# brantburnett/Snappier

Measured on AMD Instinct MI355X. Metric: uncompressed GB/s block compress+decompress, 64 KiB blocks, higher is better.
Workload: dtype u8

## Files before the change

include/snappier_hip.h:

```cpp
#ifndef SNAPPIER_HIP_H
#define SNAPPIER_HIP_H

#include <stddef.h>
#include <stdint.h>

#ifdef __cplusplus
extern "C" {
#endif

typedef enum snp_status {
    SNP_OK = 0,
    SNP_ERR_OUTPUT_TOO_SMALL = 1,
    SNP_ERR_BAD_OFFSET = 2,
    SNP_ERR_TOO_LONG = 3,
    SNP_ERR_INCOMPLETE = 4,
    SNP_ERR_BAD_LENGTH = 5,
    SNP_ERR_CRC_MISMATCH = 6,
    SNP_ERR_CHUNK_TYPE = 7,
    SNP_ERR_OVERLAP = 8,
    SNP_ERR_BAD_ARG = 9,
    SNP_ERR_DEVICE = 10,
    SNP_ERR_TRUNCATED_STREAM = 11
} snp_status;

// ... 31 lines not shown
    SNP_OPT_PARALLEL_DECODE_MIN = 8,
    SNP_OPT_FENCED = 9,
    SNP_OPT_DECODE_LEFTOVERS = 10,
    SNP_OPT_CRC_KERNEL = 11,
    SNP_OPT_COMPRESS_WINDOW_POSITIONS = 12,
    SNP_OPT_COMPRESS_WINDOW_GLOBAL_MIN_BATCH = 13,
    SNP_OPT_COMPRESS_LANE_STORES = 14,
    SNP_OPT_COMPRESS_LANE_PROBES = 15,
    SNP_OPT_COMPRESS_LANES_PER_WAVEFRONT = 16,
    SNP_OPT_COMPRESS_SLICE = 17,
    SNP_OPT_COMPRESS_SMALL_INPUT_LDS = 18,
    SNP_OPT_COMPRESS_SMALL_INPUT_LANES = 19,
    SNP_OPT_FRAME_SCAN = 20,
    SNP_OPT_DECODE_LDS_THROTTLE = 21,
    SNP_OPT_COMPRESS_WINDOW_GLOBAL_SLOTS = 22,
    SNP_OPT_COMPRESS_WINDOW_DUAL_MIN_BATCH = 23
} snp_option;
#define SNP_OPT_CRC_TABLE_FREE SNP_OPT_CRC_KERNEL
snp_status snp_ctx_set_option(snp_ctx* ctx, int option, int64_t value);
snp_status snp_ctx_get_option(const snp_ctx* ctx, int option, int64_t* out_value);
snp_status snp_ctx_reserve_compress(snp_ctx* ctx, uint32_t nfragments);
const char* snp_status_string(int status);
const char* snp_version(void);


int64_t snp_max_compressed_length(int64_t n);
int64_t snp_max_fragment_compressed_length(int64_t n);
snp_status snp_get_uncompressed_length(const uint8_t* in, size_t n, uint32_t* out_len, uint32_t* out_header_bytes);


snp_status snp_try_compress(snp_ctx* ctx, const uint8_t* in, size_t n, uint8_t* out, size_t cap, size_t* written);
// ... 50 lines not shown
```

snappier_amd/_native.py:

```python
from __future__ import annotations

import ctypes as C
import os
import re

import torch

HERE = os.path.dirname(os.path.abspath(__file__))
LIB_PATH = os.environ.get("SNAPPIER_HIP_LIB") or os.path.join(HERE, "libsnappier_hip.so")
HEADER_PATH = os.path.join(HERE, "..", "include", "snappier_hip.h")

(OK, ERR_OUTPUT_TOO_SMALL, ERR_BAD_OFFSET, ERR_TOO_LONG, ERR_INCOMPLETE, ERR_BAD_LENGTH, ERR_CRC_MISMATCH,
 ERR_CHUNK_TYPE, ERR_OVERLAP, ERR_BAD_ARG, ERR_DEVICE, ERR_TRUNCATED_STREAM) = range(12)
HASH_CRC32C, HASH_MUL = 0, 1
BLOCK_SIZE = 65536
MAX_BLOCK_COMPRESSED = 76491
(OPT_DECODE_LAYOUT, OPT_SMALL_BLOCK_MAX, OPT_SMALL_BLOCK_MIN_BATCH, OPT_COMPRESS_LAYOUT, OPT_COMPRESS_WINDOW_MAX_BATCH,
 OPT_TABLE_PROBE_TRIES, OPT_TABLE_PROBE_MAX_BYTES, OPT_PARALLEL_DECODE_MIN, OPT_FENCED, OPT_DECODE_LEFTOVERS, OPT_CRC_KERNEL,
 OPT_COMPRESS_WINDOW_POSITIONS, OPT_COMPRESS_WINDOW_GLOBAL_MIN_BATCH, OPT_COMPRESS_LANE_STORES, OPT_COMPRESS_LANE_PROBES,
 OPT_COMPRESS_LANES_PER_WAVEFRONT, OPT_COMPRESS_SLICE, OPT_COMPRESS_SMALL_INPUT_LDS, OPT_COMPRESS_SMALL_INPUT_LANES, OPT_FRAME_SCAN,
 OPT_DECODE_LDS_THROTTLE, OPT_COMPRESS_WINDOW_GLOBAL_SLOTS, OPT_COMPRESS_WINDOW_DUAL_MIN_BATCH) = range(1, 24)
OPT_CRC_TABLE_FREE = OPT_CRC_KERNEL
DECODE_AUTO, DECODE_WAVE_ONLY, DECODE_SMALL_LANES, DECODE_SMALL_TEAM4, DECODE_SMALL_TEAM8, DECODE_SMALL_TEAM16, DECODE_SERIAL = range(7)
COMPRESS_AUTO, COMPRESS_LANES, COMPRESS_WINDOW_LDS, COMPRESS_WINDOW_GLOBAL, COMPRESS_WINDOW_DUAL = 0, 2, 3, 4, 5


def declared_symbols(header: str = HEADER_PATH) -> list[str]:
    with open(header) as f:
        text = f.read()
    text = re.sub(r"/\*.*?\*/", "", text, flags=re.S)
    return sorted(set(re.findall(r"\b(snp_[a-z0-9_]+)\s*\(", text)))


_lib = None
_lab = None
LAB_PATH = os.path.join(HERE, "variants", "libsnappier_hip_lab.so")
# ... 198 lines not shown
```

snappier_amd/csrc/capi_batch.hip:

```cpp
#include "capi_internal.h"

#ifndef SNP_W_DUAL_LDS_PER_CU
#define SNP_W_DUAL_LDS_PER_CU 4u
#endif

bool snp_ctx::launch_decompress(const u8* d_in, const u64* in_off, const u32* in_len, u32 nblocks, u8* d_out, const u64* out_off,
                       const u32* out_cap, u32* out_len, i32* status, const u8* chunk_type)
{
    if (small_max && nblocks >= small_min_blocks && decode_layout == 0 && !no_prepass) {
        const u32 sub_cap = nblocks / 64 + 128;
        if (!ensure(redo, (static_cast<size_t>(sub_cap) * 64 + 128) * 4, "hipMalloc(redo list)")) return false;
        u32* const ctl = static_cast<u32*>(redo.p);
        u32* const list = ctl + 128;
        const bool capturing = stream_is_capturing();
        RelaxedCaptureMode relaxed;
        if (capturing) {
        } else if (hint && hint_ev && hint_pending && hipEventQuery(hint_ev) == hipSuccess) {
            hint_pending = false;
            if (hint_from_prepass) {
                u64 left = 0;
                for (int k = 0; k < 64; ++k) left += hint[k];
                hint_mostly_large = left * 2 > hint_blocks;
            } else if (hint[67]) {
                hint_mostly_large = static_cast<u64>(hint[65]) * 2 < hint[67];
// ... 105 lines not shown
    }
    const bool capturing = stream_is_capturing();
    if (capturing) {
    } else if (chint && chint_ev && chint_pending && hipEventQuery(chint_ev) == hipSuccess) {
        chint_pending = false;
        chint_small = chint[0] != 0 && chint[0] <= 512;
        chint_mid = chint[0] != 0 && chint[0] <= 4096;
        chint_tiny = (chint[0] > 80 && chint[0] <= 768) ? static_cast<int>((chint[0] + 15u) >> 4) : 0;
    } else {
        (void)hipGetLastError();
    }
    const u32 kSlice = slice_fragments;
    if (!ensure(small, 256, "hipMalloc(scalars)") || !borrow_tables(nblocks < kSlice ? nblocks : kSlice)) return false;
    snp_lane_tuning tune = lane_tune;
    tune.hint = (chint_small ? 32 : 0) | (chint_mid ? 256 : 0) | (chint_tiny << 9);
    for (u32 first = 0; first < nblocks; first += kSlice) {
        const u32 cnt = nblocks - first < kSlice ? nblocks - first : kSlice;
        if (!check(snp_launch_compress_lanes(d_in, in_off + first, in_len + first, cnt, d_out, out_off + first,
                                             out_len + first, status + first, variant, emit_varint, &tp,
                                             static_cast<u32*>(small.p), stream, &tune),
                   "compress (lanes) launch")) {
            return_tables();
            return false;
        }
    }
    return_tables();
    if (!capturing && chint_ready() && !chint_pending) {
        if (hipMemcpyAsync(chint, small.p, 4, hipMemcpyDeviceToHost, stream) == hipSuccess && hipEventRecord(chint_ev, stream) == hipSuccess)
            chint_pending = true;
        else
            (void)hipGetLastError();
    }
    return true;
}

bool snp_ctx::side_stream_ready()
{
    if (side_state) return side_state > 0;
    side_state = -1;
    RelaxedCaptureMode relaxed;
    if (hipStreamCreateWithFlags(&side_stream, hipStreamNonBlocking) != hipSuccess) { (void)hipGetLastError(); side_stream = nullptr; return false; }
    for (auto& e : side_ev)
        if (hipEventCreateWithFlags(&e, hipEventDisableTiming) != hipSuccess) { (void)hipGetLastError(); return false; }
    side_state = 1;
    return true;
}

bool snp_ctx::chint_ready()
{
    if (!chint && hipHostMalloc(reinterpret_cast<void**>(&chint), 64, hipHostMallocDefault) != hipSuccess) { (void)hipGetLastError(); chint = nullptr; return false; }
    if (!chint_ev && hipEventCreateWithFlags(&chint_ev, hipEventDisableTiming) != hipSuccess) { (void)hipGetLastError(); chint_ev = nullptr; return false; }
    return true;
}

extern "C" {


snp_status snp_compress_batch(snp_ctx* c, const uint8_t* in, const uint64_t* in_off, const uint32_t* in_len,
                              uint32_t nblocks, uint8_t* out, const uint64_t* out_off, uint32_t* out_len,
                              int32_t* status)
{
    if (!c || (nblocks && (!in || !in_off || !in_len || !out || !out_off || !out_len || !status))) return SNP_ERR_BAD_ARG;
// ... 39 lines not shown
```

snappier_amd/csrc/capi_ctx.hip:

```cpp
#include "capi_internal.h"

bool snp_ctx::check(hipError_t e, const char* what)
{
    if (e == hipSuccess) return true;
    err = std::string(what) + ": " + hipGetErrorString(e);
    return false;
}

bool snp_ctx::ensure(DevBuf& b, size_t bytes, const char* what)
{
    if (bytes <= b.cap) return true;
    if (stream_is_capturing()) {
        err = std::string(what) + ": a workspace would have to grow while the stream is being captured -- make the same call once before the capture (or snp_ctx_reserve_compress)";
        return false;
    }
    if (b.p) {
        if (was_captured) kept.push_back(b.p);
        else (void)hipFree(b.p);
    }
    b.p = nullptr;
    b.cap = 0;
    size_t want = bytes + bytes / 4 + 4096;
    if (!check(hipMalloc(&b.p, want), what)) return false;
    b.cap = want;
// ... 103 lines not shown
    }
    c->pool = snp_pool_of(device);
    if (!c->pool) { if (c->own_stream) (void)hipStreamDestroy(c->stream); delete c; return SNP_ERR_DEVICE; }
    {
        std::lock_guard<std::mutex> g(c->pool->mu);
        ++c->pool->users;
    }
    c->fenced = 1 | 8;
#ifdef SNAPPIER_HIP_DEBUG_ENV
    snp_apply_debug_env(c);
#endif
    *out_ctx = c;
    return SNP_OK;
}

uint64_t snp_ctx_counter(const snp_ctx* c, int which) { return (c && which >= 0 && which < 7) ? c->counters[which] : 0; }

snp_status snp_ctx_reserve_compress(snp_ctx* c, uint32_t nfragments)
{
    if (!c) return SNP_ERR_BAD_ARG;
    if (nfragments == 0) return SNP_OK;
    DevGuard dg(c);
    if (!dg.ok) return SNP_ERR_DEVICE;
    if (!c->borrow_tables(nfragments < c->slice_fragments ? nfragments : c->slice_fragments, true)) return SNP_ERR_DEVICE;
    c->return_tables();
    return SNP_OK;
}

snp_status snp_ctx_set_option(snp_ctx* c, int option, int64_t v)
{
    if (!c) return SNP_ERR_BAD_ARG;
// ... 79 lines not shown
        case SNP_OPT_COMPRESS_SMALL_INPUT_LANES:
            if (v != 0 && v != 16 && v != 32 && v != 64) return SNP_ERR_BAD_ARG;
            c->lane_tune.small_lanes = static_cast<int>(v);
            return SNP_OK;
        case SNP_OPT_FRAME_SCAN:
            if (v != 0 && v != 1) return SNP_ERR_BAD_ARG;
            c->frame_scan = static_cast<int>(v);
            return SNP_OK;
        case SNP_OPT_COMPRESS_WINDOW_GLOBAL_SLOTS:
            if (v < 0 || v > 65536) return SNP_ERR_BAD_ARG;
            c->win_gslots = static_cast<u32>(v);
            return SNP_OK;
        case SNP_OPT_COMPRESS_WINDOW_DUAL_MIN_BATCH:
            if (v < 0 || v > 0xffffffffll) return SNP_ERR_BAD_ARG;
            c->win_dual_min = static_cast<u32>(v);
            return SNP_OK;
        case SNP_OPT_DECODE_LDS_THROTTLE:
            if (v < 0 || v > 65536) return SNP_ERR_BAD_ARG;
            c->dec_lds = static_cast<int>(v / 256 * 256);
            return SNP_OK;
        default:
            return SNP_ERR_BAD_ARG;
    }
}

snp_status snp_ctx_get_option(const snp_ctx* c, int option, int64_t* out)
{
    if (!c || !out) return SNP_ERR_BAD_ARG;
    switch (option) {
        case SNP_OPT_DECODE_LAYOUT: *out = (c->fenced & 2) ? 6 : c->no_prepass ? 1 : c->small_lanes ? 2 : c->small_team_log ? c->small_team_log + 1 : 0; return SNP_OK;
// ... 7 lines not shown
        case SNP_OPT_FENCED: *out = c->fenced & 1; return SNP_OK;
        case SNP_OPT_DECODE_LEFTOVERS: *out = c->redo_grid ? 1 : c->redo_list ? 2 : 0; return SNP_OK;
        case SNP_OPT_CRC_KERNEL: *out = c->crc_kernel; return SNP_OK;
        case SNP_OPT_COMPRESS_WINDOW_POSITIONS: *out = c->win_np; return SNP_OK;
        case SNP_OPT_COMPRESS_WINDOW_GLOBAL_MIN_BATCH: *out = c->win_gtab_min; return SNP_OK;
        case SNP_OPT_COMPRESS_LANE_STORES: *out = c->lane_tune.opts; return SNP_OK;
        case SNP_OPT_COMPRESS_LANE_PROBES: *out = c->lane_tune.probes; return SNP_OK;
        case SNP_OPT_COMPRESS_LANES_PER_WAVEFRONT: *out = c->lane_tune.lanes_per_wave; return SNP_OK;
        case SNP_OPT_COMPRESS_SLICE: *out = c->slice_fragments; return SNP_OK;
        case SNP_OPT_COMPRESS_SMALL_INPUT_LDS: *out = c->lane_tune.small_bytes; return SNP_OK;
        case SNP_OPT_COMPRESS_SMALL_INPUT_LANES: *out = c->lane_tune.small_lanes; return SNP_OK;
        case SNP_OPT_FRAME_SCAN: *out = c->frame_scan; return SNP_OK;
        case SNP_OPT_DECODE_LDS_THROTTLE: *out = c->dec_lds; return SNP_OK;
        case SNP_OPT_COMPRESS_WINDOW_GLOBAL_SLOTS: *out = c->win_gslots; return SNP_OK;
        case SNP_OPT_COMPRESS_WINDOW_DUAL_MIN_BATCH: *out = c->win_dual_min; return SNP_OK;
        default: return SNP_ERR_BAD_ARG;
    }
}

void snp_ctx_destroy(snp_ctx* c)
{
    if (!c) return;
    {
        DevGuard dg(c);
        (void)hipStreamSynchronize(c->stream);
        for (DevBuf* b : {&c->in, &c->out, &c->meta, &c->work, &c->fragtab, &c->scan, &c->small, &c->redo, &c->win_tables, &c->own_tables})
            if (b->p) (void)hipFree(b->p);
        for (void* q : c->kept) (void)hipFree(q);
        if (c->pool) {
            std::lock_guard<std::mutex> g(c->pool->mu);
            if (--c->pool->users == 0) c->pool->destroy();
        }
        if (c->order_ev) (void)hipEventDestroy(c->order_ev);
        if (c->hint_ev) (void)hipEventDestroy(c->hint_ev);
        if (c->chint_ev) (void)hipEventDestroy(c->chint_ev);
        if (c->chint) (void)hipHostFree(c->chint);
        if (c->hint) (void)hipHostFree(c->hint);
        if (c->copy_stream) { (void)hipStreamSynchronize(c->copy_stream); (void)hipStreamDestroy(c->copy_stream); }
        if (c->side_stream) { (void)hipStreamSynchronize(c->side_stream); (void)hipStreamDestroy(c->side_stream); }
        for (auto& e : c->side_ev) if (e) (void)hipEventDestroy(e);
        for (auto& e : c->copy_ev) if (e) (void)hipEventDestroy(e);
        if (c->own_stream) (void)hipStreamDestroy(c->stream);
    }
    delete c;
}

snp_status snp_ctx_set_stream(snp_ctx* c, void* stream)
{
    if (!c) return SNP_ERR_BAD_ARG;
    DevGuard dg(c);
    if (!dg.ok) return SNP_ERR_DEVICE;
    hipStream_t next = static_cast<hipStream_t>(stream);
    if (c->own_stream) {
        (void)hipStreamSynchronize(c->stream);
        (void)hipStreamDestroy(c->stream);
// ... 70 lines not shown
```

snappier_amd/csrc/capi_internal.h:

```cpp
#pragma once
#include <hip/hip_runtime.h>

#include <cstdio>
#include <cstring>
#include <new>
#include <algorithm>
#include <cmath>
#include <chrono>
#include <mutex>
#include <string>
#include <utility>
#include <vector>

#include "snp_rules.h"

struct ChunkRows {
    u8* type;
    u64 *body_off, *out_off;
    u32 *body_len, *crc, *out_cap, *out_len, *tag;
    i32* status;
};

extern "C" {
hipError_t snp_launch_decompress(const u8*, const u64*, const u32*, u32, u8*, const u64*, const u32*, u32*, i32*,
                                 const u8*, int, hipStream_t, const u32*);
u32 snp_tag_index_entries(u32, u32);
size_t snp_tag_index_workspace_bytes(u32, u32);
size_t snp_tag_index_fallback_offset(u32, u32);
hipError_t snp_launch_tag_index(const u8*, u32, u32, u32, u64*, u64*, u32*, u64*, u32*, u32*, hipStream_t);
u32 snp_tag_index_chunks_ready(u32, u32, u64);
hipError_t snp_launch_tag_index_begin(u64*, u32, u32, int, hipStream_t);
int snp_tag_index_look_back_only(u32, u32);
hipError_t snp_launch_tag_index_chunks(const u8*, u32, u32, u64*, u32, u32, hipStream_t);
hipError_t snp_launch_tag_index_finish(const u8*, u32, u32, u32, u64*, u64*, u32*, u64*, u32*, u32*, hipStream_t);
hipError_t snp_launch_compress_win(const u8*, const u64*, const u32*, u32, u8*, const u64*, u32*, i32*, int, int, int,
                                   hipStream_t, uint16_t*, u32);
size_t snp_compress_win_table_bytes(u32);
hipError_t snp_launch_compress_win_dual(const u8*, const u64*, const u32*, u32, u8*, const u64*, u32*, i32*, int, int, hipStream_t, hipStream_t,
                                        hipEvent_t, hipEvent_t, uint16_t*, u32, u32, u32*);
hipError_t snp_launch_decompress_small(const u8*, const u64*, const u32*, u32, u8*, const u64*, const u32*, u32*, i32*, const u8*,
                                       u32, hipStream_t, u32*, u32*, u32, u32);
hipError_t snp_launch_sample_caps(const u32*, u32, u32, u32*, hipStream_t);
hipError_t snp_launch_decompress_list(const u8*, const u64*, const u32*, u32, u8*, const u64*, const u32*, u32*, i32*, const u8*, int,
                                      hipStream_t, const u32*, u32*, u32, u32);
hipError_t snp_launch_compress_lanes(const u8*, const u64*, const u32*, u32, u8*, const u64*, u32*, i32*, int, int, const snp_table_pieces*,
                                     u32*, hipStream_t, const snp_lane_tuning*);
size_t snp_compress_lanes_workspace(u32);
hipError_t snp_probe_tables(const snp_table_pieces*, u32, u32, hipStream_t, float*);
hipError_t snp_launch_crc32c(const u8*, const u64*, const u32*, u32, int, u32*, const u32*, i32*, hipStream_t);
hipError_t snp_launch_gather(const u8*, const u64*, const u32*, u8*, const u64*, u32, hipStream_t);
hipError_t snp_launch_frame_chunks(u64, u32, u64, u64*, u32*, u64*, hipStream_t);
hipError_t snp_launch_frame_plan(const u32*, const u32*, u32, u8*, u32*, u64*, u64*, hipStream_t);
hipError_t snp_launch_frame_header_only(u8*, u64*, hipStream_t);
hipError_t snp_launch_frame_scan(const u8*, u64, u64, u32, const ChunkRows&, u64*, hipStream_t);
// ... 58 lines not shown
    int crc_kernel = 0;
    int crc_bits() const { return crc_kernel == 1 ? 2 : crc_kernel == 2 ? 4 : 0; }
    bool no_prepass = false;
    bool small_lanes = false;
    bool redo_grid = false, redo_list = false;
    u32 small_team_log = 0;
    u32 slice_fragments = 262144;
    u32 win_gtab_min = 4096;
    u32 win_gslots = 0;
    u32 win_dual_min = 1536;
    hipStream_t side_stream = nullptr;
    hipEvent_t side_ev[2] = {nullptr, nullptr};
    int side_state = 0;
    bool side_stream_ready();
    u32 win_max = 32768;
    snp_lane_tuning lane_tune{0, -1, 0, -1, 0, 0};
    DevBuf in, out, meta, work, fragtab, scan, small, redo, win_tables;
    int frame_scan = 0;
    uint64_t counters[7] = {0, 0, 0, 0, 0, 0, 0};
    bool table_tries_set = false;
    std::string err;

    bool launch_decompress(const u8* d_in, const u64* in_off, const u32* in_len, u32 nblocks, u8* d_out, const u64* out_off,
                           const u32* out_cap, u32* out_len, i32* status, const u8* chunk_type);
    bool launch_compress(const u8* d_in, const u64* in_off, const u32* in_len, u32 nblocks, u8* d_out, const u64* out_off,
                         u32* out_len, i32* status, int emit_varint);
    bool decode_chunks(const u8* d_in, const ChunkRows& r, u32 n, u8* d_out);
    u32* hint = nullptr;
    hipEvent_t hint_ev = nullptr;
    bool hint_pending = false, hint_mostly_large = false, hint_from_prepass = false, hint_seen = false;
    u32 hint_blocks = 0, hint_mean_cap = 256;
    bool hint_ready();
    u32 n_waves = 0;
    u32 persistent_waves();
// ... 49 lines not shown
```

snappier_amd/csrc/compress_lanes.hip:

```cpp
#include <cstdlib>

#include "snp_device.h"

#ifndef SNP_CL_FLAT
#define SNP_CL_FLAT 1
#endif
#ifndef SNP_CL_SLOTS
#define SNP_CL_SLOTS 1
#endif

namespace {

constexpr u32 kDefaultSlots = SNP_CL_SLOTS;

constexpr u32 crc_step32(u32 x)
{
    for (int k = 0; k < 32; ++k) x = (x >> 1) ^ ((x & 1u) ? 0x82F63B78u : 0u);
    return x;
}

__device__ __forceinline__ u32 check_bits(u32 bytes) { return (bytes * 0x9E3779B1u) & 0xffff0000u; }

__device__ __forceinline__ u32 table_swap(u32* p, u32 v) { return __hip_atomic_exchange(p, v, __ATOMIC_RELAXED, __HIP_MEMORY_SCOPE_AGENT); }

// ... 562 lines not shown

namespace {
__global__ void k_debug_lane_match_length(const u8* buf, u32 n, u32 s1, u32 s2, u32* out)
{
    if (threadIdx.x == 0) *out = lane_find_match_length(buf, s1, s2, n);
}
}
extern "C" int snp_debug_lane_match_length(const u8* d_buf, u32 n, u32 s1, u32 s2, u32* d_out, hipStream_t stream)
{
    hipLaunchKernelGGL(k_debug_lane_match_length, dim3(1), dim3(SNP_WAVE), 0, stream, d_buf, n, s1, s2, d_out);
    return static_cast<int>(hipGetLastError());
}

extern "C" size_t snp_compress_lanes_workspace(u32 nblocks) { return static_cast<size_t>(nblocks) * 16384u * sizeof(u32); }

__global__ __launch_bounds__(256) void k_max_len(const u32* __restrict__ in_len, u32 nblocks, u32* __restrict__ max_len)
{
    u32 m = 0;
    for (u32 i = blockIdx.x * 256 + threadIdx.x; i < nblocks; i += gridDim.x * 256) m = max(m, in_len[i]);
    for (int sh = 32; sh >= 1; sh >>= 1) m = max(m, static_cast<u32>(__shfl_xor(static_cast<int>(m), sh, 64)));
    if ((threadIdx.x & 63u) == 0) atomicMax(max_len, m);
}

extern "C" hipError_t snp_launch_compress_lanes(const u8* in, const u64* in_off, const u32* in_len, u32 nblocks, u8* out,
                                                const u64* out_off, u32* out_len, i32* status, int variant,
                                                int emit_varint, const snp_table_pieces* tables, u32* max_len, hipStream_t stream, const snp_lane_tuning* tune)
{
    if (nblocks == 0) return hipSuccess;
    hipError_t e = snp_zero_words_async(max_len, 1, stream);
    if (e != hipSuccess) return e;
    const u32 mgrid = (nblocks + 255) / 256 < 1024 ? (nblocks + 255) / 256 : 1024u;
    hipLaunchKernelGGL(k_max_len, dim3(mgrid), dim3(256), 0, stream, in_len, nblocks, max_len);
    const char* env = SNP_GETENV("SNAPPIER_HIP_LANES_PER_WAVE");
    const bool two_probes = (tune->hint & 256) != 0;
    const u32 small_hint = ((static_cast<u32>(tune->hint) >> 9) & 63u) << 4;
    const u32 lanes_hint = tune->lanes_per_wave ? static_cast<u32>(tune->lanes_per_wave) : static_cast<u32>(tune->hint & 255);
    u32 per = env ? static_cast<u32>(atoi(env)) : lanes_hint ? lanes_hint : (nblocks >= 131072 ? 64u : nblocks >= 8192 ? 32u : 16u);
    if (per != 64 && per != 32 && per != 16 && per != 8) per = 64;
    const u32 grid = (nblocks + per - 1) / per;
    const char* ex = SNP_GETENV("SNAPPIER_HIP_EXACT_LITERALS");
    const char* oe = SNP_GETENV("SNAPPIER_HIP_CL_OPTS");
    const int opts = ((ex && ex[0] == '1') ? 0 : oe ? (atoi(oe) & 255) : tune->opts >= 0 ? (tune->opts & 255)
                      : ((nblocks >= 32768 ? 23 : 7) | 64 | ((nblocks >= 131072 && !two_probes) ? 128 : 0)));
    const char* se = SNP_GETENV("SNAPPIER_HIP_CL_SLOTS");
    const u32 slots = se ? static_cast<u32>(atoi(se)) : tune->probes > 0 ? static_cast<u32>(tune->probes) : ((nblocks >= 131072 && !two_probes) ? kDefaultSlots : 2u);
    const char* sm = SNP_GETENV("SNAPPIER_HIP_CL_SMALL");
    u32 small_max = sm ? (static_cast<u32>(atoi(sm)) + 15u) & ~15u : tune->small_bytes >= 0 ? (static_cast<u32>(tune->small_bytes) + 15u) & ~15u : small_hint;
    if (small_max > 2048) small_max = 0;
    if (small_max) {
        const char* sp = SNP_GETENV("SNAPPIER_HIP_CL_SMALL_PER");
        u32 sper = sp ? static_cast<u32>(atoi(sp)) : tune->small_lanes ? static_cast<u32>(tune->small_lanes) : 32u;
        if (sper != 64 && sper != 32 && sper != 16) sper = 32;
        const u32 sgrid = (nblocks + sper - 1) / sper;
        const u32 dyn = sper * (small_max + 16u + kStageStride);
        bool small_ok = true;
#define SNP_LAUNCH_SMALL(V)                                                                                                                         \
    do {                                                                                                                                            \
        if (dyn > 48u * 1024u && hipFuncSetAttribute(reinterpret_cast<const void*>(&k_compress_lanes<V, 2, true>), hipFuncAttributeMaxDynamicSharedMemorySize, static_cast<int>(dyn)) != hipSuccess) { \
            small_ok = false;                                                                                                                       \
            break;                                                                                                                                  \
// ... 5 lines not shown
        if (variant == SNP_HASH_CRC32C) SNP_LAUNCH_SMALL(SNP_HASH_CRC32C); else SNP_LAUNCH_SMALL(SNP_HASH_MUL);
#undef SNP_LAUNCH_SMALL
        if (!small_ok) {
            (void)hipGetLastError();
            small_max = 0;
        }
    }
#define SNP_LAUNCH_CL(V, S)                                                                                          \
    hipLaunchKernelGGL((k_compress_lanes<V, S, false>), dim3(grid), dim3(per), 0, stream, in, in_off, in_len, nblocks, out,    \
                       out_off, out_len, status, emit_varint, *tables, opts, max_len, small_max)
    if (variant == SNP_HASH_CRC32C) { if (slots == 1) SNP_LAUNCH_CL(SNP_HASH_CRC32C, 1); else if (slots >= 4) SNP_LAUNCH_CL(SNP_HASH_CRC32C, 4); else if (slots == 3) SNP_LAUNCH_CL(SNP_HASH_CRC32C, 3); else SNP_LAUNCH_CL(SNP_HASH_CRC32C, 2); }
    else { if (slots == 1) SNP_LAUNCH_CL(SNP_HASH_MUL, 1); else if (slots >= 4) SNP_LAUNCH_CL(SNP_HASH_MUL, 4); else if (slots == 3) SNP_LAUNCH_CL(SNP_HASH_MUL, 3); else SNP_LAUNCH_CL(SNP_HASH_MUL, 2); }
#undef SNP_LAUNCH_CL
    return hipGetLastError();
}
```

snappier_amd/csrc/compress_win.hip:

```cpp
#include <cstdlib>

#include "snp_device.h"

#ifndef SNP_W_CAP
#define SNP_W_CAP 32
#endif
#ifndef SNP_W_PROF
#define SNP_W_PROF 0
#endif
#ifndef SNP_W_PREFILTER
#define SNP_W_PREFILTER 1
#endif
#ifndef SNP_W_PREFILTER_BITS
#define SNP_W_PREFILTER_BITS 11
#endif
#ifndef SNP_W_ASMWALK
#define SNP_W_ASMWALK 1
#endif

namespace {

constexpr u32 kCap = SNP_W_CAP;
constexpr int kPieces = SNP_W_CAP / 16;
constexpr u32 kNone = 0xffffffffu;
// ... 804 lines not shown
    if ((e = hipEventRecord(fork, stream)) != hipSuccess || (e = hipStreamWaitEvent(side, fork, 0)) != hipSuccess) return e;
    const u32 g = nblocks < slots ? nblocks : slots;
    const u32 l = nblocks < lds_groups ? nblocks : lds_groups;
    if (variant == SNP_HASH_CRC32C) {
        hipLaunchKernelGGL((k_compress_win_gq<SNP_HASH_CRC32C>), dim3(g), dim3(SNP_WAVE), 0, side, in, in_off, in_len, nblocks, out, out_off, out_len, status, emit_varint, tables, ticket);
        hipLaunchKernelGGL((k_compress_win_q<SNP_HASH_CRC32C>), dim3(l), dim3(SNP_WAVE), 0, stream, in, in_off, in_len, nblocks, out, out_off, out_len, status, emit_varint, ticket);
    } else {
        hipLaunchKernelGGL((k_compress_win_gq<SNP_HASH_MUL>), dim3(g), dim3(SNP_WAVE), 0, side, in, in_off, in_len, nblocks, out, out_off, out_len, status, emit_varint, tables, ticket);
        hipLaunchKernelGGL((k_compress_win_q<SNP_HASH_MUL>), dim3(l), dim3(SNP_WAVE), 0, stream, in, in_off, in_len, nblocks, out, out_off, out_len, status, emit_varint, ticket);
    }
    if ((e = hipGetLastError()) != hipSuccess) return e;
    if ((e = hipEventRecord(join, side)) != hipSuccess) return e;
    return hipStreamWaitEvent(stream, join, 0);
}

#if SNP_W_PROF
extern "C" int snp_debug_read_wprof(unsigned long long* out16, int reset)
{
    hipError_t e = hipMemcpyFromSymbol(out16, HIP_SYMBOL(g_wprof), sizeof(g_wprof));
    if (e == hipSuccess && reset) {
        unsigned long long z[16] = {0};
        e = hipMemcpyToSymbol(HIP_SYMBOL(g_wprof), z, sizeof(z));
    }
    return static_cast<int>(e);
}
#endif

extern "C" size_t snp_compress_win_table_bytes(u32 slots) { return static_cast<size_t>(slots) * 16384u * sizeof(u16); }

extern "C" hipError_t snp_launch_compress_win(const u8* in, const u64* in_off, const u32* in_len, u32 nblocks, u8* out,
// ... 24 lines not shown
```

snappier_amd/csrc/snp_device.h:

```cpp
#pragma once
#include <hip/hip_runtime.h>
#include <stdint.h>

#include "../../include/snappier_hip.h"

typedef uint8_t u8;
typedef uint16_t u16;
typedef uint32_t u32;
typedef uint64_t u64;
typedef int32_t i32;

#define SNP_WAVE 64
#define SNP_SCAN_TILE 1024u

#ifdef SNAPPIER_HIP_DEBUG_ENV
#include <stdlib.h>
#define SNP_GETENV(name) getenv(name)
#else
#define SNP_GETENV(name) static_cast<const char*>(nullptr)
#endif

#define SNP_TABLE_PIECES_MAX 16
struct snp_table_pieces {
    uint32_t* p[SNP_TABLE_PIECES_MAX];
    uint32_t piece_frags;
    uint32_t n;
};

struct snp_lane_tuning {
    int lanes_per_wave;
    int opts;
    int probes;
    int small_bytes;
    int small_lanes;
    int hint;
};

struct __attribute__((packed)) snp_u32_unaligned { u32 v; };
struct __attribute__((packed)) snp_u64_unaligned { u64 v; };
struct __attribute__((packed)) snp_u128_unaligned { u32 v[4]; };

__device__ __forceinline__ u32 ld32u(const u8* p) { return reinterpret_cast<const snp_u32_unaligned*>(p)->v; }
__device__ __forceinline__ u64 ld64u(const u8* p) { return reinterpret_cast<const snp_u64_unaligned*>(p)->v; }
__device__ __forceinline__ void st32u(u8* p, u32 v) { reinterpret_cast<snp_u32_unaligned*>(p)->v = v; }

__device__ __forceinline__ u32 lane_id() { return __builtin_amdgcn_mbcnt_hi(~0u, __builtin_amdgcn_mbcnt_lo(~0u, 0u)); }
__device__ __forceinline__ u64 ballot64(bool p) { return __ballot(p); }
__device__ __forceinline__ u32 bcast_first(u32 v) { return __builtin_amdgcn_readfirstlane(v); }
__device__ __forceinline__ u32 read_lane(u32 v, u32 lane) { return __builtin_amdgcn_readlane(v, lane); }
__device__ __forceinline__ u64 lanes_below(u32 lane) { return lane >= 64 ? ~0ull : ((1ull << lane) - 1ull); }
// ... 67 lines not shown
```

Before: 82.52.

## Offload a tuned share of lane compression to a concurrent side-stream window kernel

Adds a sidecar path for lane-based batch compression. A fraction of fragments is sent to the window-queue compress kernel on a second stream, running alongside the lane kernel on the main stream. The split fraction is adapted online from event timings, with a later plain-run check that drops the sidecar if it does not help. Side workgroup counts are sized from LDS and occupancy probes so the lane kernel keeps its residency. This adds fork/join events, extra launches and timing overhead, and only engages by default for batches of at least 98304 fragments.

```diff
diff --git a/include/snappier_hip.h b/include/snappier_hip.h
--- a/include/snappier_hip.h
+++ b/include/snappier_hip.h
@@ -69,7 +69,9 @@
     SNP_OPT_FRAME_SCAN = 20,
     SNP_OPT_DECODE_LDS_THROTTLE = 21,
     SNP_OPT_COMPRESS_WINDOW_GLOBAL_SLOTS = 22,
-    SNP_OPT_COMPRESS_WINDOW_DUAL_MIN_BATCH = 23
+    SNP_OPT_COMPRESS_WINDOW_DUAL_MIN_BATCH = 23,
+    SNP_OPT_COMPRESS_LANE_SIDECAR = 24,
+    SNP_OPT_COMPRESS_LANE_SIDECAR_MIN_BATCH = 25
 } snp_option;
 #define SNP_OPT_CRC_TABLE_FREE SNP_OPT_CRC_KERNEL
 snp_status snp_ctx_set_option(snp_ctx* ctx, int option, int64_t value);
diff --git a/snappier_amd/_native.py b/snappier_amd/_native.py
--- a/snappier_amd/_native.py
+++ b/snappier_amd/_native.py
@@ -19,7 +19,8 @@
  OPT_TABLE_PROBE_TRIES, OPT_TABLE_PROBE_MAX_BYTES, OPT_PARALLEL_DECODE_MIN, OPT_FENCED, OPT_DECODE_LEFTOVERS, OPT_CRC_KERNEL,
  OPT_COMPRESS_WINDOW_POSITIONS, OPT_COMPRESS_WINDOW_GLOBAL_MIN_BATCH, OPT_COMPRESS_LANE_STORES, OPT_COMPRESS_LANE_PROBES,
  OPT_COMPRESS_LANES_PER_WAVEFRONT, OPT_COMPRESS_SLICE, OPT_COMPRESS_SMALL_INPUT_LDS, OPT_COMPRESS_SMALL_INPUT_LANES, OPT_FRAME_SCAN,
- OPT_DECODE_LDS_THROTTLE, OPT_COMPRESS_WINDOW_GLOBAL_SLOTS, OPT_COMPRESS_WINDOW_DUAL_MIN_BATCH) = range(1, 24)
+ OPT_DECODE_LDS_THROTTLE, OPT_COMPRESS_WINDOW_GLOBAL_SLOTS, OPT_COMPRESS_WINDOW_DUAL_MIN_BATCH, OPT_COMPRESS_LANE_SIDECAR,
+ OPT_COMPRESS_LANE_SIDECAR_MIN_BATCH) = range(1, 26)
 OPT_CRC_TABLE_FREE = OPT_CRC_KERNEL
 DECODE_AUTO, DECODE_WAVE_ONLY, DECODE_SMALL_LANES, DECODE_SMALL_TEAM4, DECODE_SMALL_TEAM8, DECODE_SMALL_TEAM16, DECODE_SERIAL = range(7)
 COMPRESS_AUTO, COMPRESS_LANES, COMPRESS_WINDOW_LDS, COMPRESS_WINDOW_GLOBAL, COMPRESS_WINDOW_DUAL = 0, 2, 3, 4, 5
diff --git a/snappier_amd/csrc/capi_batch.hip b/snappier_amd/csrc/capi_batch.hip
--- a/snappier_amd/csrc/capi_batch.hip
+++ b/snappier_amd/csrc/capi_batch.hip
@@ -143,18 +143,88 @@
     if (!ensure(small, 256, "hipMalloc(scalars)") || !borrow_tables(nblocks < kSlice ? nblocks : kSlice)) return false;
     snp_lane_tuning tune = lane_tune;
     tune.hint = (chint_small ? 32 : 0) | (chint_mid ? 256 : 0) | (chint_tiny << 9);
+    const bool side_wanted = (lane_side > 0 || (lane_side < 0 && nblocks >= lane_side_min && side_share.frac > 0.0)) &&
+                             (side_state > 0 || (!capturing && side_stream_ready()));
+    if (side_t_pending && !capturing) {
+        RelaxedCaptureMode relaxed;
+        if (hipEventQuery(side_tev[1]) == hipSuccess && (side_t_s == 0 || hipEventQuery(side_tev[2]) == hipSuccess)) {
+            side_t_pending = false;
+            float lane_ms = 0.f, side_ms = 0.f;
+            if (hipEventElapsedTime(&lane_ms, side_tev[0], side_tev[1]) == hipSuccess &&
+                (side_t_s == 0 || hipEventElapsedTime(&side_ms, side_tev[0], side_tev[2]) == hipSuccess)) {
+                if (side_t_auto && side_t_s) snp_side_share_update(side_share, side_t_n, side_t_s, lane_ms, side_ms, side_t_groups);
+                else if (side_t_auto) snp_side_share_check(side_share, side_t_n, lane_ms);
+                counters[9] = static_cast<uint64_t>(lane_ms * 1000.f);
+                counters[10] = static_cast<uint64_t>(side_ms * 1000.f);
+            } else {
+                (void)hipGetLastError();
+            }
+        } else {
+            (void)hipGetLastError();
+        }
+    }
+    const bool side_fp = side_wanted && side_footprint(nblocks < kSlice ? nblocks : kSlice, tune, capturing);
+    bool any_lane = false, timed = false;
+    counters[7] = counters[8] = 0;
     for (u32 first = 0; first < nblocks; first += kSlice) {
         const u32 cnt = nblocks - first < kSlice ? nblocks - first : kSlice;
-        if (!check(snp_launch_compress_lanes(d_in, in_off + first, in_len + first, cnt, d_out, out_off + first,
-                                             out_len + first, status + first, variant, emit_varint, &tp,
-                                             static_cast<u32*>(small.p), stream, &tune),
-                   "compress (lanes) launch")) {
+        u32 lane_n = cnt, groups = 0;
+        bool plain_check = false;
+        if (side_fp && (lane_side > 0 || cnt >= lane_side_min)) {
+            const u32 per = side_fp_per ? side_fp_per : 64u;
+            groups = side_groups_for((cnt + per - 1) / per, lane_side > 0);
+            const u32 s = lane_side > 0 ? static_cast<u32>(lane_side > 0xffffffffll ? 0xffffffffll : lane_side) : snp_side_fragments(side_share, cnt, groups);
+            plain_check = lane_side < 0 && groups && s && !timed && !capturing && !side_t_pending && snp_side_share_wants_plain(side_share) && side_timing_ready();
+            if (groups && s && !plain_check) lane_n = snp_side_lane_fragments(cnt, s);
+        }
+        const u32 side_n = cnt - lane_n;
+        u32* const ticket = static_cast<u32*>(small.p) + 32;
+        bool ok = true;
+        const bool time_it = plain_check || (side_n && lane_n && !timed && !capturing && !side_t_pending && side_timing_ready());
+        if (plain_check) {
+            tune.shape_n = 0;
+            ok = check(hipEventRecord(side_tev[0], stream), "hipEventRecord(side timing)");
+        } else if (side_n) {
+            tune.shape_n = cnt;
+            ok = check(snp_zero_words_async(ticket, 1, stream), "zero(side ticket)") &&
+                 (!time_it || check(hipEventRecord(side_tev[0], stream), "hipEventRecord(side timing)")) &&
+                 check(hipEventRecord(side_ev[0], stream), "hipEventRecord(side fork)") && check(hipStreamWaitEvent(side_stream, side_ev[0], 0), "hipStreamWaitEvent(side fork)");
+        } else {
+            tune.shape_n = 0;
+        }
+        ok = ok && check(snp_launch_compress_lanes(d_in, in_off + first, in_len + first, lane_n, d_out, out_off + first,
+                                                   out_len + first, status + first, variant, emit_varint, &tp,
+                                                   static_cast<u32*>(small.p), stream, &tune),
+                         "compress (lanes) launch");
+        if (ok && plain_check) {
+            ok = check(hipEventRecord(side_tev[1], stream), "hipEventRecord(side timing)");
+            if (ok) {
+                timed = side_t_pending = side_t_auto = true;
+                side_t_n = cnt; side_t_s = 0; side_t_groups = 0;
+            }
+        } else if (ok && side_n) {
+            const u32 at = first + lane_n;
+            ok = (!time_it || check(hipEventRecord(side_tev[1], stream), "hipEventRecord(side timing)")) &&
+                 check(snp_launch_compress_win_side(d_in, in_off + at, in_len + at, side_n, d_out, out_off + at, out_len + at, status + at, variant, emit_varint,
+                                                    side_stream, groups, ticket), "compress (side population) launch") &&
+                 (!time_it || check(hipEventRecord(side_tev[2], side_stream), "hipEventRecord(side timing)")) &&
+                 check(hipEventRecord(side_ev[1], side_stream), "hipEventRecord(side join)") && check(hipStreamWaitEvent(stream, side_ev[1], 0), "hipStreamWaitEvent(side join)");
+            if (ok && time_it) {
+                timed = side_t_pending = true;
+                side_t_auto = lane_side < 0;
+                side_t_n = cnt; side_t_s = side_n; side_t_groups = side_n < groups ? side_n : groups;
+            }
+            counters[7] += side_n;
+            counters[8] = side_n < groups ? side_n : groups;
+        }
+        if (!ok) {
             return_tables();
             return false;
         }
+        any_lane = any_lane || lane_n != 0;
     }
     return_tables();
-    if (!capturing && chint_ready() && !chint_pending) {
+    if (!capturing && any_lane && chint_ready() && !chint_pending) {
         if (hipMemcpyAsync(chint, small.p, 4, hipMemcpyDeviceToHost, stream) == hipSuccess && hipEventRecord(chint_ev, stream) == hipSuccess)
             chint_pending = true;
         else
@@ -175,6 +245,42 @@
     return true;
 }
 
+bool snp_ctx::side_timing_ready()
+{
+    if (side_tev_state) return side_tev_state > 0;
+    side_tev_state = -1;
+    RelaxedCaptureMode relaxed;
+    for (auto& e : side_tev)
+        if (hipEventCreate(&e) != hipSuccess) { (void)hipGetLastError(); e = nullptr; return false; }
+    side_tev_state = 1;
+    return true;
+}
+
+bool snp_ctx::side_footprint(u32 shape_n, const snp_lane_tuning& t, bool capturing)
+{
+    const u32 cls = shape_n >= 131072 ? 3u : shape_n >= 32768 ? 2u : shape_n >= 8192 ? 1u : 0u;
+    const u32 key = cls | (static_cast<u32>(t.lanes_per_wave) << 2) | (static_cast<u32>(t.probes) << 10) | ((static_cast<u32>(t.hint) & 0x1ffu) << 13);
+    if (key == side_fp_key || (capturing && side_fp_key != 0xffffffffu)) return true;
+    if (capturing) return false;
+    int lds = 0;
+    if (hipDeviceGetAttribute(&lds, hipDeviceAttributeMaxSharedMemoryPerMultiprocessor, device) != hipSuccess || lds <= 0) { (void)hipGetLastError(); return false; }
+    u32 per = 0, lane_lds = 0, lane_occ = 0, win_lds = 0;
+    if (snp_probe_lanes_footprint(variant, shape_n, &t, &per, &lane_lds, &lane_occ) != hipSuccess || snp_probe_win_side_lds(variant, &win_lds) != hipSuccess) {
+        (void)hipGetLastError();
+        return false;
+    }
+    side_fp_key = key; side_fp_per = per; side_fp_lane_lds = lane_lds; side_fp_lane_occ = lane_occ; side_fp_win_lds = win_lds; side_fp_lds_cu = static_cast<u32>(lds);
+    return true;
+}
+
+u32 snp_ctx::side_groups_for(u32 lane_groups, bool forced)
+{
+    const u32 cus = persistent_waves() / 32u;
+    u32 k = snp_side_groups_per_cu(side_fp_lds_cu, side_fp_lane_lds, side_fp_win_lds, side_fp_lane_occ, cus, lane_groups);
+    if (k == 0 && forced) k = 1;
+    return k * cus;
+}
+
 bool snp_ctx::chint_ready()
 {
     if (!chint && hipHostMalloc(reinterpret_cast<void**>(&chint), 64, hipHostMallocDefault) != hipSuccess) { (void)hipGetLastError(); chint = nullptr; return false; }
diff --git a/snappier_amd/csrc/capi_ctx.hip b/snappier_amd/csrc/capi_ctx.hip
--- a/snappier_amd/csrc/capi_ctx.hip
+++ b/snappier_amd/csrc/capi_ctx.hip
@@ -141,7 +141,7 @@
     return SNP_OK;
 }
 
-uint64_t snp_ctx_counter(const snp_ctx* c, int which) { return (c && which >= 0 && which < 7) ? c->counters[which] : 0; }
+uint64_t snp_ctx_counter(const snp_ctx* c, int which) { return (c && which >= 0 && which < 11) ? c->counters[which] : 0; }
 
 snp_status snp_ctx_reserve_compress(snp_ctx* c, uint32_t nfragments)
 {
@@ -251,6 +251,14 @@
         case SNP_OPT_COMPRESS_WINDOW_DUAL_MIN_BATCH:
             if (v < 0 || v > 0xffffffffll) return SNP_ERR_BAD_ARG;
             c->win_dual_min = static_cast<u32>(v);
+            return SNP_OK;
+        case SNP_OPT_COMPRESS_LANE_SIDECAR:
+            if (v < -1 || v > 0xffffffffll) return SNP_ERR_BAD_ARG;
+            c->lane_side = v;
+            return SNP_OK;
+        case SNP_OPT_COMPRESS_LANE_SIDECAR_MIN_BATCH:
+            if (v < 0 || v > 0xffffffffll) return SNP_ERR_BAD_ARG;
+            c->lane_side_min = static_cast<u32>(v);
             return SNP_OK;
         case SNP_OPT_DECODE_LDS_THROTTLE:
             if (v < 0 || v > 65536) return SNP_ERR_BAD_ARG;
@@ -288,6 +296,8 @@
         case SNP_OPT_DECODE_LDS_THROTTLE: *out = c->dec_lds; return SNP_OK;
         case SNP_OPT_COMPRESS_WINDOW_GLOBAL_SLOTS: *out = c->win_gslots; return SNP_OK;
         case SNP_OPT_COMPRESS_WINDOW_DUAL_MIN_BATCH: *out = c->win_dual_min; return SNP_OK;
+        case SNP_OPT_COMPRESS_LANE_SIDECAR: *out = c->lane_side; return SNP_OK;
+        case SNP_OPT_COMPRESS_LANE_SIDECAR_MIN_BATCH: *out = c->lane_side_min; return SNP_OK;
         default: return SNP_ERR_BAD_ARG;
     }
 }
@@ -313,6 +323,7 @@
         if (c->copy_stream) { (void)hipStreamSynchronize(c->copy_stream); (void)hipStreamDestroy(c->copy_stream); }
         if (c->side_stream) { (void)hipStreamSynchronize(c->side_stream); (void)hipStreamDestroy(c->side_stream); }
         for (auto& e : c->side_ev) if (e) (void)hipEventDestroy(e);
+        for (auto& e : c->side_tev) if (e) (void)hipEventDestroy(e);
         for (auto& e : c->copy_ev) if (e) (void)hipEventDestroy(e);
         if (c->own_stream) (void)hipStreamDestroy(c->stream);
     }
diff --git a/snappier_amd/csrc/capi_internal.h b/snappier_amd/csrc/capi_internal.h
--- a/snappier_amd/csrc/capi_internal.h
+++ b/snappier_amd/csrc/capi_internal.h
@@ -13,6 +13,7 @@
 #include <vector>
 
 #include "snp_rules.h"
+#include "lane_side_share.h"
 
 struct ChunkRows {
     u8* type;
@@ -38,6 +39,9 @@
 size_t snp_compress_win_table_bytes(u32);
 hipError_t snp_launch_compress_win_dual(const u8*, const u64*, const u32*, u32, u8*, const u64*, u32*, i32*, int, int, hipStream_t, hipStream_t,
                                         hipEvent_t, hipEvent_t, uint16_t*, u32, u32, u32*);
+hipError_t snp_launch_compress_win_side(const u8*, const u64*, const u32*, u32, u8*, const u64*, u32*, i32*, int, int, hipStream_t, u32, u32*);
+hipError_t snp_probe_win_side_lds(int, u32*);
+hipError_t snp_probe_lanes_footprint(int, u32, const snp_lane_tuning*, u32*, u32*, u32*);
 hipError_t snp_launch_decompress_small(const u8*, const u64*, const u32*, u32, u8*, const u64*, const u32*, u32*, i32*, const u8*,
                                        u32, hipStream_t, u32*, u32*, u32, u32);
 hipError_t snp_launch_sample_caps(const u32*, u32, u32, u32*, hipStream_t);
@@ -126,10 +130,22 @@
     int side_state = 0;
     bool side_stream_ready();
     u32 win_max = 32768;
-    snp_lane_tuning lane_tune{0, -1, 0, -1, 0, 0};
+    snp_lane_tuning lane_tune{0, -1, 0, -1, 0, 0, 0};
+    int64_t lane_side = -1;
+    u32 lane_side_min = 98304;
+    snp_side_share side_share;
+    hipEvent_t side_tev[3] = {nullptr, nullptr, nullptr};
+    int side_tev_state = 0;
+    bool side_t_auto = false;
+    bool side_t_pending = false;
+    u32 side_t_n = 0, side_t_s = 0, side_t_groups = 0;
+    u32 side_fp_key = 0xffffffffu, side_fp_per = 0, side_fp_lane_lds = 0, side_fp_lane_occ = 0, side_fp_win_lds = 0, side_fp_lds_cu = 0;
+    bool side_timing_ready();
+    bool side_footprint(u32 shape_n, const snp_lane_tuning& tune, bool capturing);
+    u32 side_groups_for(u32 lane_groups, bool forced);
     DevBuf in, out, meta, work, fragtab, scan, small, redo, win_tables;
     int frame_scan = 0;
-    uint64_t counters[7] = {0, 0, 0, 0, 0, 0, 0};
+    uint64_t counters[11] = {0, 0, 0, 0, 0, 0, 0, 0, 0, 0, 0};
     bool table_tries_set = false;
     std::string err;
 
diff --git a/snappier_amd/csrc/compress_lanes.hip b/snappier_amd/csrc/compress_lanes.hip
--- a/snappier_amd/csrc/compress_lanes.hip
+++ b/snappier_amd/csrc/compress_lanes.hip
@@ -600,6 +600,27 @@
 
 extern "C" size_t snp_compress_lanes_workspace(u32 nblocks) { return static_cast<size_t>(nblocks) * 16384u * sizeof(u32); }
 
+struct LaneShape {
+    u32 per, slots;
+    int opts;
+    bool two_probes;
+};
+static LaneShape lane_shape(u32 shape_n, const snp_lane_tuning* tune)
+{
+    const char* env = SNP_GETENV("SNAPPIER_HIP_LANES_PER_WAVE");
+    const bool two_probes = (tune->hint & 256) != 0;
+    const u32 lanes_hint = tune->lanes_per_wave ? static_cast<u32>(tune->lanes_per_wave) : static_cast<u32>(tune->hint & 255);
+    u32 per = env ? static_cast<u32>(atoi(env)) : lanes_hint ? lanes_hint : (shape_n >= 131072 ? 64u : shape_n >= 8192 ? 32u : 16u);
+    if (per != 64 && per != 32 && per != 16 && per != 8) per = 64;
+    const char* ex = SNP_GETENV("SNAPPIER_HIP_EXACT_LITERALS");
+    const char* oe = SNP_GETENV("SNAPPIER_HIP_CL_OPTS");
+    const int opts = ((ex && ex[0] == '1') ? 0 : oe ? (atoi(oe) & 255) : tune->opts >= 0 ? (tune->opts & 255)
+                      : ((shape_n >= 32768 ? 23 : 7) | 64 | ((shape_n >= 131072 && !two_probes) ? 128 : 0)));
+    const char* se = SNP_GETENV("SNAPPIER_HIP_CL_SLOTS");
+    const u32 slots = se ? static_cast<u32>(atoi(se)) : tune->probes > 0 ? static_cast<u32>(tune->probes) : ((shape_n >= 131072 && !two_probes) ? kDefaultSlots : 2u);
+    return LaneShape{per, slots, opts, two_probes};
+}
+
 __global__ __launch_bounds__(256) void k_max_len(const u32* __restrict__ in_len, u32 nblocks, u32* __restrict__ max_len)
 {
     u32 m = 0;
@@ -617,19 +638,11 @@
     if (e != hipSuccess) return e;
     const u32 mgrid = (nblocks + 255) / 256 < 1024 ? (nblocks + 255) / 256 : 1024u;
     hipLaunchKernelGGL(k_max_len, dim3(mgrid), dim3(256), 0, stream, in_len, nblocks, max_len);
-    const char* env = SNP_GETENV("SNAPPIER_HIP_LANES_PER_WAVE");
-    const bool two_probes = (tune->hint & 256) != 0;
+    const LaneShape shp = lane_shape(tune->shape_n ? tune->shape_n : nblocks, tune);
+    const u32 per = shp.per, slots = shp.slots;
+    const int opts = shp.opts;
+    const u32 grid = (nblocks + per - 1) / per;
     const u32 small_hint = ((static_cast<u32>(tune->hint) >> 9) & 63u) << 4;
-    const u32 lanes_hint = tune->lanes_per_wave ? static_cast<u32>(tune->lanes_per_wave) : static_cast<u32>(tune->hint & 255);
-    u32 per = env ? static_cast<u32>(atoi(env)) : lanes_hint ? lanes_hint : (nblocks >= 131072 ? 64u : nblocks >= 8192 ? 32u : 16u);
-    if (per != 64 && per != 32 && per != 16 && per != 8) per = 64;
-    const u32 grid = (nblocks + per - 1) / per;
-    const char* ex = SNP_GETENV("SNAPPIER_HIP_EXACT_LITERALS");
-    const char* oe = SNP_GETENV("SNAPPIER_HIP_CL_OPTS");
-    const int opts = ((ex && ex[0] == '1') ? 0 : oe ? (atoi(oe) & 255) : tune->opts >= 0 ? (tune->opts & 255)
-                      : ((nblocks >= 32768 ? 23 : 7) | 64 | ((nblocks >= 131072 && !two_probes) ? 128 : 0)));
-    const char* se = SNP_GETENV("SNAPPIER_HIP_CL_SLOTS");
-    const u32 slots = se ? static_cast<u32>(atoi(se)) : tune->probes > 0 ? static_cast<u32>(tune->probes) : ((nblocks >= 131072 && !two_probes) ? kDefaultSlots : 2u);
     const char* sm = SNP_GETENV("SNAPPIER_HIP_CL_SMALL");
     u32 small_max = sm ? (static_cast<u32>(atoi(sm)) + 15u) & ~15u : tune->small_bytes >= 0 ? (static_cast<u32>(tune->small_bytes) + 15u) & ~15u : small_hint;
     if (small_max > 2048) small_max = 0;
@@ -665,3 +678,22 @@
 #undef SNP_LAUNCH_CL
     return hipGetLastError();
 }
+
+extern "C" hipError_t snp_probe_lanes_footprint(int variant, u32 shape_n, const snp_lane_tuning* tune, u32* per_out, u32* lds_bytes, u32* groups_per_cu)
+{
+    const LaneShape shp = lane_shape(shape_n, tune);
+    const void* fn;
+#define SNP_CL_FN(V, S) reinterpret_cast<const void*>(&k_compress_lanes<V, S, false>)
+    if (variant == SNP_HASH_CRC32C) fn = shp.slots == 1 ? SNP_CL_FN(SNP_HASH_CRC32C, 1) : shp.slots >= 4 ? SNP_CL_FN(SNP_HASH_CRC32C, 4) : shp.slots == 3 ? SNP_CL_FN(SNP_HASH_CRC32C, 3) : SNP_CL_FN(SNP_HASH_CRC32C, 2);
+    else fn = shp.slots == 1 ? SNP_CL_FN(SNP_HASH_MUL, 1) : shp.slots >= 4 ? SNP_CL_FN(SNP_HASH_MUL, 4) : shp.slots == 3 ? SNP_CL_FN(SNP_HASH_MUL, 3) : SNP_CL_FN(SNP_HASH_MUL, 2);
+#undef SNP_CL_FN
+    hipFuncAttributes a{};
+    hipError_t e = hipFuncGetAttributes(&a, fn);
+    if (e != hipSuccess) return e;
+    int groups = 0;
+    if ((e = hipOccupancyMaxActiveBlocksPerMultiprocessor(&groups, fn, static_cast<int>(shp.per), 0)) != hipSuccess) return e;
+    *per_out = shp.per;
+    *lds_bytes = static_cast<u32>(a.sharedSizeBytes);
+    *groups_per_cu = groups > 0 ? static_cast<u32>(groups) : 0u;
+    return hipSuccess;
+}
diff --git a/snappier_amd/csrc/compress_win.hip b/snappier_amd/csrc/compress_win.hip
--- a/snappier_amd/csrc/compress_win.hip
+++ b/snappier_amd/csrc/compress_win.hip
@@ -842,6 +842,28 @@
     return hipStreamWaitEvent(stream, join, 0);
 }
 
+extern "C" hipError_t snp_launch_compress_win_side(const u8* in, const u64* in_off, const u32* in_len, u32 nblocks, u8* out,
+                                                   const u64* out_off, u32* out_len, i32* status, int variant, int emit_varint,
+                                                   hipStream_t side, u32 groups, u32* ticket)
+{
+    if (nblocks == 0) return hipSuccess;
+    const u32 l = nblocks < groups ? nblocks : groups ? groups : 1u;
+    if (variant == SNP_HASH_CRC32C)
+        hipLaunchKernelGGL((k_compress_win_q<SNP_HASH_CRC32C>), dim3(l), dim3(SNP_WAVE), 0, side, in, in_off, in_len, nblocks, out, out_off, out_len, status, emit_varint, ticket);
+    else
+        hipLaunchKernelGGL((k_compress_win_q<SNP_HASH_MUL>), dim3(l), dim3(SNP_WAVE), 0, side, in, in_off, in_len, nblocks, out, out_off, out_len, status, emit_varint, ticket);
+    return hipGetLastError();
+}
+
+extern "C" hipError_t snp_probe_win_side_lds(int variant, u32* lds_bytes)
+{
+    hipFuncAttributes a{};
+    const hipError_t e = hipFuncGetAttributes(&a, variant == SNP_HASH_CRC32C ? reinterpret_cast<const void*>(&k_compress_win_q<SNP_HASH_CRC32C>)
+                                                                             : reinterpret_cast<const void*>(&k_compress_win_q<SNP_HASH_MUL>));
+    if (e == hipSuccess) *lds_bytes = static_cast<u32>(a.sharedSizeBytes);
+    return e;
+}
+
 #if SNP_W_PROF
 extern "C" int snp_debug_read_wprof(unsigned long long* out16, int reset)
 {
diff --git a/snappier_amd/csrc/lane_side_share.h b/snappier_amd/csrc/lane_side_share.h
--- /dev/null
+++ b/snappier_amd/csrc/lane_side_share.h
@@ -0,0 +1,83 @@
+#pragma once
+#include <stdint.h>
+
+constexpr uint32_t kSnpSideQuantum = 64;
+constexpr double kSnpSideFirst = 1.0 / 16;
+constexpr double kSnpSideTarget = 0.9;
+constexpr double kSnpSideStepMax = 1.25;
+constexpr double kSnpSideStepMin = 0.75;
+constexpr uint32_t kSnpSideCapDiv = 8;
+
+constexpr double kSnpSideSettled = 0.10;
+constexpr double kSnpSideMinGain = 0.01;
+
+enum snp_side_phase : int {
+    SNP_SIDE_TUNING = 0,
+    SNP_SIDE_CHECK = 1,
+    SNP_SIDE_KEPT = 2,
+};
+struct snp_side_share {
+    double frac = kSnpSideFirst;
+    int phase = SNP_SIDE_TUNING;
+    double split_ms_per_fragment = 0.0;
+};
+
+inline uint32_t snp_side_lane_fragments(uint32_t n, uint32_t s)
+{
+    return s >= n ? 0u : (n - s) / kSnpSideQuantum * kSnpSideQuantum;
+}
+
+inline uint32_t snp_side_fragments(const snp_side_share& st, uint32_t n, uint32_t side_groups)
+{
+    if (!(st.frac > 0.0)) return 0u;
+    const uint64_t q = static_cast<uint64_t>(st.frac * static_cast<double>(n) / kSnpSideQuantum + 0.5);
+    uint64_t s = q * kSnpSideQuantum;
+    const uint64_t cap = static_cast<uint64_t>(n / kSnpSideCapDiv) / kSnpSideQuantum * kSnpSideQuantum;
+    if (s > cap) s = cap;
+    return s < side_groups || s == 0 ? 0u : static_cast<uint32_t>(s);
+}
+
+inline void snp_side_share_update(snp_side_share& st, uint32_t n, uint32_t s, double lane_ms, double side_ms, uint32_t side_groups)
+{
+    if (!(lane_ms > 0.0) || !(side_ms > 0.0) || !(lane_ms < 1e9) || !(side_ms < 1e9) || s == 0 || s >= n) return;
+    const double rl = lane_ms / static_cast<double>(n - s), rs = side_ms / static_cast<double>(s);
+    const double want = kSnpSideTarget * static_cast<double>(n) * rl / (rs + kSnpSideTarget * rl);
+    if (want < static_cast<double>(side_groups) || want < 1.0) {
+        st.frac = 0.0;
+        return;
+    }
+    double step = want / static_cast<double>(s);
+    if (step > kSnpSideStepMax) step = kSnpSideStepMax;
+    if (step < kSnpSideStepMin) step = kSnpSideStepMin;
+    double frac = static_cast<double>(s) * step / static_cast<double>(n);
+    if (frac > 1.0 / kSnpSideCapDiv) frac = 1.0 / kSnpSideCapDiv;
+    st.frac = frac;
+    st.split_ms_per_fragment = (lane_ms > side_ms ? lane_ms : side_ms) / static_cast<double>(n);
+    if (st.phase == SNP_SIDE_TUNING && step >= 1.0 - kSnpSideSettled && step <= 1.0 + kSnpSideSettled) st.phase = SNP_SIDE_CHECK;
+}
+
+inline bool snp_side_share_wants_plain(const snp_side_share& st) { return st.phase == SNP_SIDE_CHECK && st.frac > 0.0; }
+
+inline void snp_side_share_check(snp_side_share& st, uint32_t n, double plain_ms)
+{
+    if (st.phase != SNP_SIDE_CHECK || !(plain_ms > 0.0) || !(plain_ms < 1e9) || n == 0) return;
+    if (st.split_ms_per_fragment > 0.0 && st.split_ms_per_fragment <= (1.0 - kSnpSideMinGain) * plain_ms / static_cast<double>(n)) st.phase = SNP_SIDE_KEPT;
+    else st.frac = 0.0;
+}
+
+inline uint32_t snp_side_groups_per_cu(uint32_t lds_per_cu, uint32_t lane_lds, uint32_t side_lds, uint32_t lane_occ, uint32_t cus, uint32_t lane_groups)
+{
+    if (!lds_per_cu || !side_lds || !cus) return 0u;
+    const uint32_t unit = lds_per_cu / 128u ? lds_per_cu / 128u : 1u;
+    const uint32_t lane_a = (lane_lds + unit - 1) / unit * unit, side_a = (side_lds + unit - 1) / unit * unit;
+    const uint64_t need = (static_cast<uint64_t>(lane_groups) + cus - 1) / cus;
+    uint32_t best = 0;
+    for (uint32_t k = 1; static_cast<uint64_t>(k) * side_a <= lds_per_cu; ++k) {
+        const uint32_t by_lds = lane_a ? (lds_per_cu - k * side_a) / lane_a : 0xffffffffu;
+        const uint32_t by_occ = lane_occ > k ? lane_occ - k : 0u;
+        const uint32_t room = by_lds < by_occ ? by_lds : by_occ;
+        if (room >= need) best = k;
+        else break;
+    }
+    return best;
+}
diff --git a/snappier_amd/csrc/snp_device.h b/snappier_amd/csrc/snp_device.h
--- a/snappier_amd/csrc/snp_device.h
+++ b/snappier_amd/csrc/snp_device.h
@@ -34,6 +34,7 @@
     int small_bytes;
     int small_lanes;
     int hint;
+    uint32_t shape_n;
 };
 
 struct __attribute__((packed)) snp_u32_unaligned { u32 v; };
```

Measured after the change: 81.43. 0.987x the previous value.
